# dhillon24/3d-shape-generation

Measured on AMD Instinct MI355X. Metric: denoising-steps/sec (whole node), 2048-pt DDPM, batch 64, higher is better.
Workload: dtype f16; 1 GPU; BASELINE configs[1]: point-cloud DDPM (sample2), 2048 points, batch 64 per GPU, 1000-step cosine schedule, fp16 operands/fp32 accumulate, random-init synthetic weights, denoiser UNetPointNetLarge; batch_per_gpu=64, points=2048, sampler=ddpm/sample2, backbone=pointnet, launch=eager, rccl_ranks=1

## Files before the change

3d-shape-generation_amd/_lib.py:

```python
from __future__ import annotations

import ctypes as C
import os
import subprocess
from typing import Optional

_HERE = os.path.dirname(os.path.abspath(__file__))
LIB_PATH = os.path.join(_HERE, "libpcd_hip.so")
ABI_VERSION = 2
CSRC = os.path.join(_HERE, "csrc")

vp = C.c_void_p
i32, i64, u64, f32, sz = C.c_int, C.c_int64, C.c_uint64, C.c_float, C.c_size_t

PCD_UNET_NLIN = 26


class GemmDesc(C.Structure):
    _fields_ = [("a1", vp), ("lda1", i64), ("k1", i32),
                ("a2", vp), ("lda2", i64), ("k2", i32),
                ("w", vp), ("ldw", i64),
                ("bias", vp), ("shape_bias", vp), ("rows_per_shape", i32),
                ("relu", i32), ("m", i32), ("c", i32)]

# ... 65 lines not shown


class VaeConvT(C.Structure):
    _fields_ = [("w", vp * 8), ("taps", vp * 8), ("b", vp), ("cin", i32), ("cout", i32)]


class VaeDesc(C.Structure):
    _fields_ = [("latent_dim", i32), ("enc0_w", vp), ("enc0_b", vp),
                ("enc_res", VaeRes * 4), ("enc_down", VaeConv * 3), ("enc_last", VaeConv),
                ("fc_w", vp), ("fc_b", vp), ("din_w", vp), ("din_b", vp),
                ("dec_up", VaeConvT * 3), ("dec_res", VaeRes * 4), ("dec_conv9", VaeConv),
                ("last_w", vp), ("last_b", f32),
                ("taps3", vp), ("taps4s2", vp), ("taps4p0", vp), ("taps1", vp), ("zero_page", vp)]


class RenderStyle(C.Structure):
    _fields_ = [("colors", vp), ("light", f32 * 3), ("ambient", f32), ("background", f32 * 3)]


PCD_PAIR_WS = ("an", "bn", "mins", "alpha", "beta", "rowc", "cmax", "err", "bits", "total")


def pair_metrics_workspace_layout(pairs: int, na_max: int, nb_max: int) -> dict:
    off = (sz * len(PCD_PAIR_WS))()
    check(load().pcd_pair_metrics_workspace_layout(pairs, na_max, nb_max, off), "pair_metrics_workspace_layout")
    return dict(zip(PCD_PAIR_WS, (int(v) for v in off)))


PCD_SURF_ROW = ("ACC", "COMP", "CHAMFER_L1", "ACC2", "COMP2", "CHAMFER_L2", "HAUSDORFF", "NC_A", "NC_B", "NC")
PCD_SURF_ROW_BASE = len(PCD_SURF_ROW)
PCD_SURF_MAX_THRESHOLDS = 8
PCD_KNN_MAX_K = 32
PCD_NORMALS_UNORIENTED, PCD_NORMALS_OUTWARD, PCD_NORMALS_TOWARD_VIEW = 0, 1, 2
PCD_OUTLIER_STATISTICAL, PCD_OUTLIER_RADIUS = 0, 1


_SIGS = {
    "pcd_last_error": (C.c_char_p, []),
    "pcd_abi_version": (i32, []),
    "pcd_device_check": (i32, []),
    "pcd_gemm_f16": (i32, [C.POINTER(GemmDesc), vp, i64, vp]),
    "pcd_gemm_f16_hilo": (i32, [C.POINTER(GemmDesc), vp, i64, vp]),
    "pcd_gemm_f16_out32": (i32, [C.POINTER(GemmDesc), vp, i64, vp]),
    "pcd_gemm_f16_splitk": (i32, [C.POINTER(GemmDesc), i32, vp, vp]),
    "pcd_sum_slabs_f32": (i32, [vp, i32, i64, i32, vp, i64, vp]),
    "pcd_gemm_f16_residual": (i32, [C.POINTER(GemmDesc), vp, i64, vp, i64, vp]),
    "pcd_gemm_f16_colmax": (i32, [C.POINTER(GemmDesc), vp, i32, vp]),
    "pcd_gemm_pack_wfrag": (i32, [vp, i64, i32, i32, vp, vp]),
    "pcd_gemm_f16_colmax_wfrag": (i32, [C.POINTER(GemmDesc), vp, vp, i32, vp]),
    "pcd_gemm_wfrag_enabled": (i32, []),
    "pcd_gemm_f16_wfrag": (i32, [C.POINTER(GemmDesc), vp, vp, i64, vp]),
    "pcd_gemm_store_wfrag_enabled": (i32, []),
    "pcd_gemm_wfrag_stamps": (i32, [vp]),
    "pcd_gemm_set_config": (i32, [i32]),
    "pcd_gemm_plan": (i32, [C.POINTER(GemmDesc), i32, i32, i32, i32, C.POINTER(GemmPlan)]),
    "pcd_fill_zero": (i32, [vp, sz, vp]),
    "pcd_f32_to_f16": (i32, [vp, vp, i64, vp]),
    "pcd_f16_to_f32": (i32, [vp, vp, i64, vp]),
    "pcd_time_embed": (i32, [vp, i32, vp, i32, i32, vp, vp, vp, vp, vp, vp, vp, i32, vp, vp]),
    "pcd_linear_f32": (i32, [vp, i32, i32, vp, vp, i32, vp, vp]),
    "pcd_enc1_xyz": (i32, [vp, i64, i32, vp, i32, vp, i32, vp, vp]),
    "pcd_add_noise": (i32, [vp, vp, vp, vp, i32, i64, i64, vp, vp]),
    "pcd_remove_noise": (i32, [vp, vp, vp, vp, i32, i64, i64, vp, vp]),
    "pcd_ddim_update": (i32, [vp, vp, vp, vp, vp, vp, i32, i64, i64, vp, vp, vp]),
    "pcd_ddpm_update": (i32, [vp, vp, vp, vp, vp, vp, vp, i32, i64, i64, vp, vp, vp]),
    "pcd_ddpm_update_philox": (i32, [vp, vp, vp, vp, vp, vp, i32, i64, i64, vp, vp, u64, u64, u64, vp, vp]),
    "pcd_randn": (i32, [vp, i64, u64, u64, vp]),
    "pcd_step_select": (i32, [vp, i32, vp, i32, vp, vp, i32, vp, vp]),
    "pcd_randn_step": (i32, [vp, i64, u64, u64, u64, vp, vp]),
    "pcd_step_select_cols": (i32, [vp, i32, vp, i32, vp, vp, i32, i32, vp, vp]),
    "pcd_step_select_labels": (i32, [vp, i32, vp, i32, vp, vp, i32, vp, i32, i32, vp, i32, i32, vp, vp]),
    "pcd_cfg_combine": (i32, [vp, vp, vp, i32, i64, i64, vp]),
    "pcd_complete_start": (i32, [vp, vp, vp, vp, vp, i32, i64, i64, i32, vp]),
    "pcd_complete_update": (i32, [vp, vp, vp, vp, vp, vp, vp, i32, i32, i64, i64, i32, vp, vp, vp]),
    "pcd_complete_update_philox": (i32, [vp, vp, vp, vp, vp, i32, i32, i64, i64, i32, i32, vp, vp, u64, u64, u64, u64, vp, vp]),
    "pcd_dpm_update": (i32, [vp, vp, vp, i32, i32, i64, i64, vp, vp, vp]),
    "pcd_head3": (i32, [vp, i64, i32, vp, vp, vp, vp]),
    "pcd_pw_chain_enc1": (i32, [vp, i64, i32, vp, vp, i32, vp, vp, vp, vp, vp, vp]),
    "pcd_pw_chain_enc1_hilo": (i32, [vp, i64, i32, vp, vp, i32, vp, vp, vp, vp, vp, vp]),
    "pcd_pw_chain_tail_hilo": (i32, [vp, i64, vp, vp, vp, vp, vp, vp, vp, vp, vp, vp]),
    "pcd_pw_chain_128": (i32, [vp, i64, vp, vp, vp, vp, vp, vp]),
    "pcd_pw_chain_tail": (i32, [vp, i64, vp, vp, vp, vp, vp, vp, vp, vp, vp, vp]),
    "pcd_unet_config": (i32, [i32]),
    "pcd_pw_wide_packed_bytes": (sz, [i32]),
    "pcd_pw_wide_pack": (i32, [i32, vp, vp, vp, vp]),
    "pcd_pw_wide_chain": (i32, [i32, vp, vp, i64, vp, vp, vp]),
    "pcd_pw_wide_ends_packed_bytes": (sz, [i32, i32]),
    "pcd_pw_wide_ends_pack": (i32, [i32, i32, vp, vp, vp, vp]),
    "pcd_pw_wide_ends": (i32, [i32, i32, vp, vp, vp, i64, vp, vp, vp, vp]),
    "pcd_conv1x1_supported": (i32, [i32, i32]),
    "pcd_conv1x1_f16": (i32, [vp, i64, i32, vp, i64, vp, i32, i32, vp, vp]),
    "pcd_unet_create": (i32, [C.POINTER(UnetDesc), C.POINTER(vp)]),
    "pcd_unet_destroy": (None, [vp]),
    "pcd_unet_workspace_bytes": (sz, [i32, i32]),
    "pcd_unet_forward": (i32, [vp, vp, i32, i32, vp, i32, vp, vp, sz, vp]),
    "pcd_unet_profile": (i32, [vp, i32]),
    "pcd_unet_profile_read": (i32, [vp, C.POINTER(C.c_double), C.POINTER(i32)]),
    "pcd_unet_tap": (i32, [vp, C.c_char_p, i32, i32, vp, vp, sz, vp]),
    "pcd_unet_capture": (i32, [vp, vp, vp, vp, vp]),
    "pcd_gemm_f32": (i32, [vp, i64, i32, vp, i64, i32, vp, i64, vp, vp, i32, i32, i32, i32, vp, i64, vp]),
    "pcd_gemm_f32_colmax": (i32, [vp, i64, i32, vp, i64, vp, i32, i32, vp, i32, vp]),
    "pcd_unet_f32_create": (i32, [C.POINTER(UnetDesc), C.POINTER(vp)]),
    "pcd_unet_f32_destroy": (None, [vp]),
    "pcd_unet_f32_workspace_bytes": (sz, [i32, i32]),
    "pcd_unet_f32_forward": (i32, [vp, vp, i32, i32, vp, i32, vp, vp, sz, vp]),
    "pcd_unet_f32_tap": (i32, [vp, C.c_char_p, i32, i32, vp, vp, sz, vp]),
    "pcd_unet_f32_round_activations": (i32, [vp, C.c_uint]),
    "pcd_groupnorm_relu_f16": (i32, [vp, i32, i32, i32, vp, vp, vp, vp]),
    "pcd_skinny_slabs": (i32, [i32, i32]),
    "pcd_skinny_gemm_f16": (i32, [vp, i32, vp, i32, vp, i64, i32, i32, vp, vp]),
    "pcd_skinny_gemm_f32in": (i32, [vp, i32, vp, i64, i32, i32, vp, vp]),
    "pcd_skinny_finish":(i32, [vp, i32, i32, i32, vp, vp, i32, i32, vp, vp, vp, vp, vp]),
    "pcd_skinny_config": (i32, [i32]),
    "pcd_skinny_fused_supported": (i32, [i32, i32, i32, i32]),
    "pcd_skinny_fused": (i32, [vp, i32, vp, i32, vp, i64, i32, i32, vp, vp, i32, i32, vp, vp, vp, vp, vp]),
    "pcd_skinny_fused_f32in": (i32, [vp, i32, vp, i64, i32, i32, vp, vp, i32, i32, vp, vp, vp, vp, vp]),
    "pcd_latent_create": (i32, [C.POINTER(LatentDesc), C.POINTER(vp)]),
    "pcd_latent_destroy": (None, [vp]),
    "pcd_latent_workspace_bytes": (sz, [i32]),
    "pcd_latent_forward": (i32, [vp, vp, i32, vp, i32, vp, vp, sz, vp]),
    "pcd_latent_f32_create": (i32, [C.POINTER(LatentDesc), C.POINTER(vp)]),
    "pcd_latent_f32_destroy": (None, [vp]),
    "pcd_latent_f32_workspace_bytes": (sz, [i32]),
    "pcd_latent_f32_forward": (i32, [vp, vp, i32, vp, i32, vp, vp, sz, vp]),
    "pcd_latent_persist_supported": (i32, [i32]),
    "pcd_latent_persist_create": (i32, [C.POINTER(LatentDesc), C.POINTER(vp)]),
    "pcd_latent_persist_destroy": (None, [vp]),
    "pcd_latent_persist_workspace_bytes": (sz, [vp]),
    "pcd_latent_persist_config": (i32, [vp, i32, i32]),
    "pcd_latent_persist_trace": (i32, [vp, vp, i32]),
    "pcd_latent_persist_forward": (i32, [vp, vp, i32, vp, vp, vp, sz, vp]),
    "pcd_latent_persist_ddim": (i32, [vp, vp, vp, i32, vp, i32, vp, i32, i32, vp, i32, vp, sz, vp]),
    "pcd_latent_persist_status": (i32, [vp, C.POINTER(C.c_uint), vp]),
    "pcd_latent_persist_inject_fault": (i32, [vp, i32, i32]),
    "pcd_latent_persist_plan_check": (i32, []),
    "pcd_latent_persist_plan_dump": (i32, [vp]),
    "pcd_conv3d_f16": (i32, [C.POINTER(Conv3dDesc), vp]),
    "pcd_conv3d_k3s1_supported": (i32, [C.POINTER(Conv3dDesc)]),
    "pcd_conv3d_k3s1_f16": (i32, [C.POINTER(Conv3dDesc), vp]),
    "pcd_conv3d_workspace_bytes": (sz, [C.POINTER(Conv3dDesc), i32]),
    "pcd_conv3d_f16_multi": (i32, [C.POINTER(Conv3dDesc), i32, vp, sz, vp]),
    "pcd_conv3d_wfrag_bytes": (sz, [i32, i32]),
    "pcd_conv3d_pack_wfrag": (i32, [vp, i32, i32, i32, i32, vp, vp]),
    "pcd_conv3d_k3s1_wreg_supported": (i32, [C.POINTER(Conv3dDesc)]),
    "pcd_conv3d_k3s1_wreg_f16": (i32, [C.POINTER(Conv3dDesc), vp, vp]),
    "pcd_conv3d_k4s2_halo_supported": (i32, [i32, i32, i32, i32, i32, i32, i32]),
    "pcd_conv3d_k4s2_halo_f16": (i32, [vp, i32, i32, i32, i32, i32, vp, i32, vp, i32, i32, vp, vp]),
    "pcd_convt3d_k4s2_halo_supported": (i32, [i32, i32, i32, i32, i32, i32]),
    "pcd_convt3d_k4s2_halo_f16": (i32, [vp, i32, i32, i32, i32, i32, C.POINTER(vp), vp, i32, vp, vp]),
    "pcd_conv3d_first": (i32, [vp, i32, i32, i32, i32, i32, vp, vp, i32, vp, vp]),
    "pcd_convt3d_last_sigmoid": (i32, [vp, i32, i32, i32, i32, i32, vp, f32, vp, vp]),
    "pcd_conv3d_config": (i32, [i32]),
    "pcd_conv3d_last_sigmoid": (i32, [vp, i32, i32, i32, i32, i32, vp, f32, vp, vp]),
    "pcd_conv3d_last_packed_bytes": (sz, []),
    "pcd_conv3d_last_pack": (i32, [vp, vp, vp]),
    "pcd_conv3d_last_sigmoid_packed": (i32, [vp, i32, i32, i32, i32, i32, vp, vp, f32, vp, vp]),
    "pcd_reparameterize": (i32, [vp, vp, vp, vp, i64, vp]),
    "pcd_vae_config": (i32, [i32]),
    "pcd_vae_create": (i32, [C.POINTER(VaeDesc), C.POINTER(vp)]),
    "pcd_vae_destroy": (None, [vp]),
    "pcd_vae_workspace_bytes": (sz, [i32]),
    "pcd_vae_encode": (i32, [vp, vp, i32, vp, vp, sz, vp]),
    "pcd_vae_decode": (i32, [vp, vp, i32, vp, vp, sz, vp]),
    "pcd_layernorm_f16": (i32, [vp, i64, i32, vp, vp, vp, vp]),
    "pcd_set_attention_workspace_bytes": (sz, [i32, i32, i32]),
    "pcd_set_attention_f16": (i32, [vp, i32, i32, i32, i32, vp, vp, sz, vp]),
# ... 178 lines not shown
```

3d-shape-generation_amd/csrc/unet.hip:

```cpp
#include <string.h>
#include <new>
#include "common.h"

struct pcd_unet {
    pcd_unet_desc_t d;
    static constexpr int kMaxEv = 4096;
    int prof_on = 0;
    int prof_n = 0;
    hipEvent_t ev0[kMaxEv];
    hipEvent_t ev1[kMaxEv];
    int ev_created = 0;
    void* wide[2] = {nullptr, nullptr};
    void* ends[2] = {nullptr, nullptr};
    void* gf3_frag = nullptr;
    void* lin_frag[PCD_UNET_NLIN] = {};
    void* dec_tap[4] = {nullptr, nullptr, nullptr, nullptr};
};

namespace pcd {

int pw_chain_enc1_impl(const float* x, int64_t m, int rows_per_shape, const float* w_xyz, const float* tbias, int tbias_shape_stride,
                       const void* w_conv2, const float* b_conv2, const void* w_conv3, const float* b_conv3, void* x1, bool hilo,
                       float* zero, int64_t zero_n, void* stream);


struct UnetWs {
    size_t x1, x2, x3, x4, s0, s1, pooled, pooled16, gbias, total;
};

static UnetWs carve(int64_t batch, int64_t n) {
    const size_t m = (size_t)batch * (size_t)n;
    UnetWs w{};
    size_t o = 0;
    w.x1 = o; o += align_up(m * 128 * 2);
    w.x2 = o; o += align_up(m * 256 * 2);
    w.x3 = o; o += align_up(m * 512 * 2);
    w.x4 = o; o += align_up(m * 1024 * 2);
    w.s0 = o; o += align_up(m * 2048 * 2);
    const size_t slabs = batch <= 256 ? (size_t)pcd_skinny_slabs(4096, 1024) * (size_t)batch * 1024 * 4 : 0;
    w.s1 = o; o += align_up(m * 1024 * 2 > slabs ? m * 1024 * 2 : slabs);
    w.pooled = o; o += align_up((size_t)batch * 4096 * 4);
    w.pooled16 = o; if (batch > 256) o += align_up((size_t)batch * 4096 * 2);
    w.gbias = o; o += align_up((size_t)batch * 1024 * 4);
    w.total = o;
    return w;
}

}

using namespace pcd;

static const int kLinK[PCD_UNET_NLIN] = {64, 64, 128, 128, 128, 256, 256, 256, 512, 512, 512, 1024, 2048,
                                         1024, 1024, 1024, 1024, 512, 512, 512, 256, 256, 256, 128, 128, 64};
static const int kLinC[PCD_UNET_NLIN] = {64, 128, 128, 128, 256, 256, 256, 512, 512, 512, 1024, 2048, 4096,
                                         1024, 1024, 512, 512, 512, 256, 256, 256, 128, 128, 128, 64, 64};

static int g_unet_chains = 3;

extern "C" int pcd_unet_config(int use_chains) {
    g_unet_chains = use_chains & 3;
    return PCD_OK;
}

extern "C" int pcd_unet_create(const pcd_unet_desc_t* desc, pcd_unet_t** out) {
    PCD_CHECK_ARG(desc != nullptr && out != nullptr);
    PCD_CHECK_ARG(desc->freqs && desc->tw0 && desc->tb0 && desc->tw2 && desc->tb2);
    PCD_CHECK_ARG(desc->e1w_xyz && desc->e1w_t && desc->e1b && desc->wg && desc->head_w && desc->head_b);
    PCD_CHECK_ARG(desc->wg_k == 4096 && desc->wg_c == 1024);
    if (desc->hilo_mask & ~PCD_UNET_HILO_ALLOWED) {
        set_error("pcd_unet_create: hilo_mask 0x%x names layers outside 0x%x", desc->hilo_mask, PCD_UNET_HILO_ALLOWED);
        return PCD_ERR_ARG;
    }
    for (int i = 0; i < PCD_UNET_NLIN; ++i) {
        if (desc->lin[i].w == nullptr || desc->lin[i].b == nullptr || desc->lin[i].k != kLinK[i] ||
            desc->lin[i].c != kLinC[i]) {
            set_error("pcd_unet_create: layer %d expects %d->%d, got %d->%d (or null pointers)", i, kLinK[i],
                      kLinC[i], desc->lin[i].k, desc->lin[i].c);
            return PCD_ERR_ARG;
        }
    }
    pcd_unet* h = new (std::nothrow) pcd_unet;
    PCD_CHECK_ARG(h != nullptr);
    h->d = *desc;
    const int first[2] = {5, 19};
    for (int c = 0; c < 2; ++c) {
        const void* w[3] = {desc->lin[first[c]].w, desc->lin[first[c] + 1].w, desc->lin[first[c] + 2].w};
        const float* b[3] = {desc->lin[first[c]].b, desc->lin[first[c] + 1].b, desc->lin[first[c] + 2].b};
        hipError_t e = hipMalloc(&h->wide[c], pcd_pw_wide_packed_bytes(c));
        int rc = e == hipSuccess ? pcd_pw_wide_pack(c, w, b, h->wide[c], nullptr) : PCD_ERR_HIP;
        if (rc == PCD_OK && hipStreamSynchronize(nullptr) != hipSuccess) rc = PCD_ERR_HIP;
        if (rc != PCD_OK) {
            if (e != hipSuccess) set_error("pcd_unet_create: %s", hipGetErrorString(e));
            pcd_unet_destroy(h);
            return rc;
        }
    }
    h->gf3_frag = pcd_packed_copy(desc->lin[12].w, (size_t)4096 * 2048 * 2,
                                  [&](void* buf) { return pcd_gemm_pack_wfrag(desc->lin[12].w, 2048, 2048, 4096, buf, nullptr); });
    for (int i = 8; i <= 18; ++i) {
        if (i == 12 || ((desc->hilo_mask >> i) & 1u) || kLinK[i] < 384 || kLinC[i] % 256 != 0) continue;
        h->lin_frag[i] = pcd_packed_copy(desc->lin[i].w, (size_t)kLinK[i] * kLinC[i] * 2,
                                         [&](void* buf) { return pcd_gemm_pack_wfrag(desc->lin[i].w, kLinK[i], kLinK[i], kLinC[i], buf, nullptr); });
    }
    for (int c = 0; c < 2; ++c) {
        const int first = c == 0 ? 2 : 19, nl = c == 0 ? 6 : 4;
        const int hilo = (int)((desc->hilo_mask >> (c == 0 ? 4 : 22)) & 1u);
        const void* w[6]; const float* b[6];
        for (int i = 0; i < nl; ++i) { w[i] = desc->lin[first + i].w; b[i] = desc->lin[first + i].b; }
        h->ends[c] = pcd_packed_copy(w[0], pcd_pw_wide_ends_packed_bytes(c, hilo), [&](void* buf) { return pcd_pw_wide_ends_pack(c, hilo, w, b, buf, nullptr); });
    }
    *out = h;
    return PCD_OK;
}

extern "C" void pcd_unet_destroy(pcd_unet_t* h) {
    if (h == nullptr) return;
    if (h->gf3_frag) (void)hipFree(h->gf3_frag);
    for (int i = 0; i < PCD_UNET_NLIN; ++i) if (h->lin_frag[i]) (void)hipFree(h->lin_frag[i]);
    for (int k = 0; k < 2; ++k) if (h->wide[k]) (void)hipFree(h->wide[k]);
    for (int k = 0; k < 2; ++k) if (h->ends[k]) (void)hipFree(h->ends[k]);
    for (int i = 0; i < h->ev_created; ++i) { (void)hipEventDestroy(h->ev0[i]); (void)hipEventDestroy(h->ev1[i]); }
    delete h;
}

extern "C" int pcd_unet_profile(pcd_unet_t* h, int enable) {
    PCD_CHECK_ARG(h != nullptr);
    h->prof_on = enable ? 1 : 0;
    h->prof_n = 0;
    return PCD_OK;
}

extern "C" int pcd_unet_profile_read(pcd_unet_t* h, double* total_ms, int* launches) {
    PCD_CHECK_ARG(h && total_ms && launches);
    double tot = 0.0;
    for (int i = 0; i < h->prof_n; ++i) {
        PCD_CHECK_HIP(hipEventSynchronize(h->ev1[i]));
        float ms = 0.f;
        PCD_CHECK_HIP(hipEventElapsedTime(&ms, h->ev0[i], h->ev1[i]));
        tot += ms;
    }
    *total_ms = tot;
    *launches = h->prof_n;
    return PCD_OK;
// ... 2 lines not shown
extern "C" int pcd_unet_capture(pcd_unet_t* h, void* d4, void* d3, void* d2, void* d1) {
    PCD_CHECK_ARG(h != nullptr);
    h->dec_tap[0] = d4; h->dec_tap[1] = d3; h->dec_tap[2] = d2; h->dec_tap[3] = d1;
    return PCD_OK;
}

extern "C" size_t pcd_unet_workspace_bytes(int batch, int n_points) {
    if (batch <= 0 || n_points <= 0) return 0;
    return carve(batch, n_points).total;
}

static int run_lin(const pcd_unet_desc_t& d, int idx, int64_t m, const void* a1, const void* a2, int k2,
                   const float* shape_bias, int rps, void* out, hipStream_t s, const void* wfrag = nullptr) {
    pcd_gemm_desc_t g{};
    const pcd_linear_desc_t& L = d.lin[idx];
    g.a1 = a1; g.k1 = L.k - k2; g.lda1 = g.k1;
    g.a2 = a2; g.k2 = k2; g.lda2 = k2;
    const bool hilo = (d.hilo_mask >> idx) & 1u;
    g.w = L.w; g.ldw = hilo ? 2 * L.k : L.k;
    g.bias = shape_bias ? nullptr : L.b;
    g.shape_bias = shape_bias; g.rows_per_shape = rps;
    g.relu = 1; g.m = (int)m; g.c = L.c;
    if (hilo) return pcd_gemm_f16_hilo(&g, out, L.c, s);
    return wfrag != nullptr ? pcd_gemm_f16_wfrag(&g, wfrag, out, L.c, s) : pcd_gemm_f16(&g, out, L.c, s);
}

extern "C" int pcd_unet_forward(pcd_unet_t* h, const float* x, int batch, int n_points, const float* tbias,
                                int tbias_shape_stride, float* eps, void* workspace, size_t workspace_bytes,
                                void* stream) {
    PCD_CHECK_ARG(h && x && tbias && eps && workspace);
    PCD_CHECK_ARG(batch > 0 && n_points > 0);
    const int64_t m = (int64_t)batch * n_points;
    PCD_CHECK_ARG(m <= 0x7fffffff);
    const UnetWs w = carve(batch, n_points);
    if (workspace_bytes < w.total) {
        set_error("pcd_unet_forward: workspace %zu < required %zu", workspace_bytes, w.total);
        return PCD_ERR_WORKSPACE;
    }
    char* ws = (char*)workspace;
    void *x1 = ws + w.x1, *x2 = ws + w.x2, *x3 = ws + w.x3, *x4 = ws + w.x4, *s0 = ws + w.s0, *s1 = ws + w.s1;
    float* pooled = (float*)(ws + w.pooled);
    float* gbias = (float*)(ws + w.gbias);
    hipStream_t s = (hipStream_t)stream;
    const pcd_unet_desc_t& d = h->d;
    int rc;
    const bool chains = (g_unet_chains & 1) != 0;
    bool pooled_cleared = false;
    const bool wide = (g_unet_chains & 2) != 0 && m % 256 == 0;
    const bool e23 = wide && h->ends[0] != nullptr;
    const bool d21 = wide && h->ends[1] != nullptr && h->dec_tap[2] == nullptr;
    if (chains) {
        const unsigned e1 = d.hilo_mask & 3u;
        if (e1 == 3u || e1 == 0u) {
            PCD_RUN(pw_chain_enc1_impl(x, m, n_points, d.e1w_xyz, tbias, tbias_shape_stride, d.lin[0].w, d.lin[0].b, d.lin[1].w, d.lin[1].b, x1,
                                   e1 == 3u, pooled, (int64_t)batch * 4096, s));
            pooled_cleared = true;
        } else {
            PCD_RUN(pcd_enc1_xyz(x, m, n_points, d.e1w_xyz, 64, tbias, tbias_shape_stride, s0, s));
            PCD_RUN(run_lin(d, 0, m, s0, nullptr, 0, nullptr, 0, s1, s));
            PCD_RUN(run_lin(d, 1, m, s1, nullptr, 0, nullptr, 0, x1, s));
        }
        if (!e23) PCD_RUN(pcd_pw_chain_128(x1, m, d.lin[2].w, d.lin[2].b, d.lin[3].w, d.lin[3].b, s1, s));
    } else {
        PCD_RUN(pcd_enc1_xyz(x, m, n_points, d.e1w_xyz, 64, tbias, tbias_shape_stride, s0, s));
        PCD_RUN(run_lin(d, 0, m, s0, nullptr, 0, nullptr, 0, s1, s));
        PCD_RUN(run_lin(d, 1, m, s1, nullptr, 0, nullptr, 0, x1, s));
        if (!e23) {
            PCD_RUN(run_lin(d, 2, m, x1, nullptr, 0, nullptr, 0, s0, s));
            PCD_RUN(run_lin(d, 3, m, s0, nullptr, 0, nullptr, 0, s1, s));
        }
    }
    if (e23) {
        PCD_RUN(pcd_pw_wide_ends(0, (int)((d.hilo_mask >> 4) & 1u), x1, nullptr, nullptr, m, h->ends[0], x3, x2, s));
    } else {
        PCD_RUN(run_lin(d, 4, m, s1, nullptr, 0, nullptr, 0, x2, s));
        if (wide) {
            PCD_RUN(pcd_pw_wide_chain(0, x2, nullptr, m, h->wide[0], x3, s));
        } else {
            PCD_RUN(run_lin(d, 5, m, x2, nullptr, 0, nullptr, 0, s0, s));
            PCD_RUN(run_lin(d, 6, m, s0, nullptr, 0, nullptr, 0, s1, s));
            PCD_RUN(run_lin(d, 7, m, s1, nullptr, 0, nullptr, 0, x3, s));
        }
    }
    PCD_RUN(run_lin(d, 8, m, x3, nullptr, 0, nullptr, 0, s0, s, h->lin_frag[8]));
    PCD_RUN(run_lin(d, 9, m, s0, nullptr, 0, nullptr, 0, s1, s, h->lin_frag[9]));
    PCD_RUN(run_lin(d, 10, m, s1, nullptr, 0, nullptr, 0, x4, s, h->lin_frag[10]));
    PCD_RUN(run_lin(d, 11, m, x4, nullptr, 0, nullptr, 0, s0, s, h->lin_frag[11]));
    {
        if (!pooled_cleared) PCD_RUN(pcd_fill_zero(pooled, (size_t)batch * 4096 * sizeof(float), s));
        pcd_gemm_desc_t g{};
        g.a1 = s0; g.k1 = 2048; g.lda1 = 2048; g.w = d.lin[12].w; g.ldw = 2048; g.bias = d.lin[12].b;
        g.relu = 1; g.m = (int)m; g.c = 4096;
        const bool prof = h->prof_on && h->prof_n < pcd_unet::kMaxEv;
        if (prof) {
            if (h->prof_n >= h->ev_created) {
                PCD_CHECK_HIP(hipEventCreate(&h->ev0[h->ev_created]));
                PCD_CHECK_HIP(hipEventCreate(&h->ev1[h->ev_created]));
                ++h->ev_created;
            }
            PCD_CHECK_HIP(hipEventRecord(h->ev0[h->prof_n], s));
        }
        if (gemm_colmax_takes_wfrag(&g, n_points, h->gf3_frag))
            PCD_RUN(pcd_gemm_f16_colmax_wfrag(&g, h->gf3_frag, pooled, n_points, s));
        else
            PCD_RUN(pcd_gemm_f16_colmax(&g, pooled, n_points, s));
        if (prof) { PCD_CHECK_HIP(hipEventRecord(h->ev1[h->prof_n], s)); ++h->prof_n; }
    }
    {
        if (batch <= 256) {
            PCD_RUN(pcd_skinny_gemm_f32in(pooled, 4096, d.wg, 4096, batch, 1024, (float*)s1, s));
            PCD_RUN(pcd_skinny_finish((const float*)s1, pcd_skinny_slabs(4096, 1024), batch, 1024, d.lin[13].b, nullptr, 2, 8,
                                  nullptr, nullptr, nullptr, gbias, s));
        } else {
            void* pooled16 = ws + w.pooled16;
            PCD_RUN(pcd_f32_to_f16(pooled, pooled16, (int64_t)batch * 4096, s));
            pcd_gemm_desc_t g{};
            g.a1 = pooled16; g.k1 = 4096; g.lda1 = 4096; g.w = d.wg; g.ldw = 4096; g.bias = d.lin[13].b;
            g.relu = 0; g.m = batch; g.c = 1024;
            PCD_RUN(pcd_gemm_f16_out32(&g, gbias, 1024, s));
        }
    }
    PCD_RUN(run_lin(d, 13, m, x4, nullptr, 0, gbias, n_points, s1, s, h->lin_frag[13]));
    PCD_RUN(run_lin(d, 14, m, s1, nullptr, 0, nullptr, 0, s0, s, h->lin_frag[14]));
    PCD_RUN(run_lin(d, 15, m, s0, nullptr, 0, nullptr, 0, s1, s, h->lin_frag[15]));
#define TAP(i, buf, ch) do { if (h->dec_tap[i]) PCD_CHECK_HIP(hipMemcpyAsync(h->dec_tap[i], buf, (size_t)m * (ch) * 2, \
                                                                             hipMemcpyDeviceToDevice, s)); } while (0)
    TAP(0, s1, 512);
    PCD_RUN(run_lin(d, 16, m, s1, x3, 512, nullptr, 0, s0, s, h->lin_frag[16]));
    PCD_RUN(run_lin(d, 17, m, s0, nullptr, 0, nullptr, 0, s1, s, h->lin_frag[17]));
    PCD_RUN(run_lin(d, 18, m, s1, nullptr, 0, nullptr, 0, s0, s, h->lin_frag[18]));
    TAP(1, s0, 256);
    void *ta = s0, *tb = s1;
    if (d21) {
        PCD_RUN(pcd_pw_wide_ends(1, (int)((d.hilo_mask >> 22) & 1u), s0, x2, x1, m, h->ends[1], s1, nullptr, s));
        ta = s1; tb = s0;
    } else {
        if (wide) {
            PCD_RUN(pcd_pw_wide_chain(1, s0, x2, m, h->wide[1], s1, s));
        } else {
            PCD_RUN(run_lin(d, 19, m, s0, x2, 256, nullptr, 0, s1, s));
            PCD_RUN(run_lin(d, 20, m, s1, nullptr, 0, nullptr, 0, s0, s));
            PCD_RUN(run_lin(d, 21, m, s0, nullptr, 0, nullptr, 0, s1, s));
        }
        TAP(2, s1, 128);
        PCD_RUN(run_lin(d, 22, m, s1, x1, 128, nullptr, 0, s0, s));
    }
    const unsigned tl = (d.hilo_mask >> 23) & 7u;
    if (chains && h->dec_tap[3] == nullptr && (tl == 0u || tl == 7u)) {
        if (tl == 7u)
            PCD_RUN(pcd_pw_chain_tail_hilo(ta, m, d.lin[23].w, d.lin[23].b, d.lin[24].w, d.lin[24].b, d.lin[25].w, d.lin[25].b, d.head_w,
                                       d.head_b, eps, s));
        else
            PCD_RUN(pcd_pw_chain_tail(ta, m, d.lin[23].w, d.lin[23].b, d.lin[24].w, d.lin[24].b, d.lin[25].w, d.lin[25].b, d.head_w,
                                  d.head_b, eps, s));
    } else {
        PCD_RUN(run_lin(d, 23, m, ta, nullptr, 0, nullptr, 0, tb, s));
        PCD_RUN(run_lin(d, 24, m, tb, nullptr, 0, nullptr, 0, ta, s));
        TAP(3, ta, 64);
        PCD_RUN(run_lin(d, 25, m, ta, nullptr, 0, nullptr, 0, tb, s));
        PCD_RUN(pcd_head3(tb, m, 64, d.head_w, d.head_b, eps, s));
    }
#undef TAP
    return PCD_OK;
}

extern "C" int pcd_unet_tap(pcd_unet_t* h, const char* name, int batch, int n_points, const void* workspace,
                            void* dst, size_t dst_bytes, void* stream) {
    PCD_CHECK_ARG(h && name && workspace && dst && batch > 0 && n_points > 0);
    const UnetWs w = carve(batch, n_points);
    const size_t m = (size_t)batch * n_points;
    size_t off = 0, bytes = 0;
    if (!strcmp(name, "x1")) { off = w.x1; bytes = m * 128 * 2; }
    else if (!strcmp(name, "x2")) { off = w.x2; bytes = m * 256 * 2; }
    else if (!strcmp(name, "x3")) { off = w.x3; bytes = m * 512 * 2; }
    else if (!strcmp(name, "x4")) { off = w.x4; bytes = m * 1024 * 2; }
    else if (!strcmp(name, "pooled")) { off = w.pooled; bytes = (size_t)batch * 4096 * 4; }
    else if (!strcmp(name, "gbias")) { off = w.gbias; bytes = (size_t)batch * 1024 * 4; }
    else { set_error("pcd_unet_tap: unknown tap '%s'", name); return PCD_ERR_ARG; }
    PCD_CHECK_ARG(dst_bytes >= bytes);
    PCD_CHECK_HIP(hipMemcpyAsync(dst, (const char*)workspace + off, bytes, hipMemcpyDeviceToDevice, (hipStream_t)stream));
    return PCD_OK;
}
```

include/pcd_hip.h:

```cpp
#ifndef PCD_HIP_H
#define PCD_HIP_H

#include <stddef.h>
#include <stdint.h>

#ifdef __cplusplus
extern "C" {
#endif

#define PCD_OK 0
#define PCD_ERR_ARG (-1)
#define PCD_ERR_HIP (-2)
#define PCD_ERR_WORKSPACE (-3)

#define PCD_ABI_VERSION 2

const char* pcd_last_error(void);
int pcd_abi_version(void);
int pcd_device_check(void);

typedef struct {
    const void* a1; int64_t lda1; int k1;
    const void* a2; int64_t lda2; int k2;
    const void* w;  int64_t ldw;
// ... 48 lines not shown
                   float* y, void* stream);

int pcd_enc1_xyz(const float* x, int64_t m, int rows_per_shape, const float* w_xyz, int c1,
                 const float* tbias, int tbias_shape_stride, void* out, void* stream);

int pcd_add_noise(const float* x0, const float* noise, const float* n, const float* s, int stride,
                  int64_t total, int64_t per_shape, float* x_t, void* stream);
int pcd_remove_noise(const float* x_t, const float* eps, const float* n, const float* s, int stride,
                     int64_t total, int64_t per_shape, float* x0, void* stream);
int pcd_ddim_update(const float* x, const float* eps, const float* n, const float* s,
                    const float* n2, const float* s2, int stride,
                    int64_t total, int64_t per_shape, float* x0, float* x_next, void* stream);
int pcd_ddpm_update(const float* x, const float* eps, const float* z, const float* n, const float* s,
                    const float* coef, const float* s2, int stride,
                    int64_t total, int64_t per_shape, float* x0, float* x_next, void* stream);
int pcd_ddpm_update_philox(const float* x, const float* eps, const float* n, const float* s, const float* coef, const float* s2,
                           int stride, int64_t total, int64_t per_shape, float* x0, float* x_next, uint64_t seed,
                           uint64_t base_offset, uint64_t per_step_stride, const int* counter, void* stream);
int pcd_randn(float* out, int64_t n, uint64_t seed, uint64_t offset, void* stream);

int pcd_step_select(int* counter, int n_steps, const float* tb_table, int tb_elems, float* tb_cur,
                    const float* rate_tables, int width, float* rates_cur, void* stream);
int pcd_randn_step(float* out, int64_t n, uint64_t seed, uint64_t base_offset, uint64_t per_step_stride,
                   const int* counter, void* stream);
int pcd_step_select_cols(int* counter, int n_steps, const float* tb_table, int tb_elems, float* tb_cur,
                         const float* rate_tables, int cols, int width, float* rates_cur, void* stream);

int pcd_step_select_labels(int* counter, int n_steps, const float* tb_table, int tb_elems, float* tb_rows,
                           const float* class_bias, int class_rows, const int* labels, int batch, int null_row,
                           const float* rate_tables, int cols, int width, float* rates_cur, void* stream);
int pcd_cfg_combine(float* eps, const float* eps_u, const float* w, int w_stride, int64_t n, int64_t per_shape, void* stream);

int pcd_complete_start(float* x, const float* p, const int* counts, const float* n, const float* s, int stride,
                       int64_t total, int64_t per_shape, int row_elems, void* stream);
int pcd_complete_update(const float* x, const float* eps, const float* z, const float* z2, const float* p,
                        const int* counts, const float* rates, int width, int stride, int64_t total,
                        int64_t per_shape, int row_elems, float* x0, float* x_next, void* stream);
int pcd_complete_update_philox(const float* x, const float* eps, const float* p, const int* counts,
                               const float* rates, int width, int stride, int64_t total, int64_t per_shape,
                               int row_elems, int jumps, float* x0, float* x_next, uint64_t seed,
                               uint64_t base_offset, uint64_t per_step_stride, uint64_t z2_offset,
                               const int* counter, void* stream);

int pcd_dpm_update(const float* x, const float* eps, const float* rates, int width, int stride, int64_t total,
                   int64_t per_shape, float* hist, float* x_next, void* stream);

int pcd_head3(const void* h, int64_t m, int k, const float* w, const float* b, float* eps, void* stream);

#define PCD_UNET_NLIN 26
typedef struct {
    const void* w; const float* b; int k; int c;
} pcd_linear_desc_t;

typedef struct {
    int time_dim, dim;
    const float* freqs;
    const float *tw0, *tb0, *tw2, *tb2;
    const float* e1w_xyz;
    const float* e1w_t;
    const float* e1b;
    pcd_linear_desc_t lin[PCD_UNET_NLIN];
    const void* wg; int wg_k, wg_c;
    const float* head_w; const float* head_b;
    unsigned hilo_mask;
} pcd_unet_desc_t;
#define PCD_UNET_HILO_ALLOWED 0x3C00013u

int pcd_pw_chain_enc1(const float* x, int64_t m, int rows_per_shape, const float* w_xyz, const float* tbias,
                      int tbias_shape_stride, const void* w_conv2, const float* b_conv2, const void* w_conv3,
                      const float* b_conv3, void* x1, void* stream);
int pcd_pw_chain_128(const void* in, int64_t m, const void* w_a, const float* b_a, const void* w_b, const float* b_b,
                     void* out, void* stream);
int pcd_pw_chain_tail(const void* in, int64_t m, const void* w_a, const float* b_a, const void* w_b, const float* b_b,
                      const void* w_c, const float* b_c, const float* head_w, const float* head_b, float* eps, void* stream);
int pcd_pw_chain_enc1_hilo(const float* x, int64_t m, int rows_per_shape, const float* w_xyz, const float* tbias,
                           int tbias_shape_stride, const void* w_conv2, const float* b_conv2, const void* w_conv3,
                           const float* b_conv3, void* x1, void* stream);
int pcd_pw_chain_tail_hilo(const void* in, int64_t m, const void* w_a, const float* b_a, const void* w_b, const float* b_b,
                           const void* w_c, const float* b_c, const float* head_w, const float* head_b, float* eps, void* stream);
int pcd_conv1x1_supported(int k, int c);
int pcd_conv1x1_f16(const void* in, int64_t m, int k, const void* w, int64_t ldw, const float* bias, int relu, int c,
                    void* out, void* stream);
int pcd_unet_config(int use_chains);
size_t pcd_pw_wide_packed_bytes(int chain);
int pcd_pw_wide_pack(int chain, const void* const* w, const float* const* b, void* packed, void* stream);
int pcd_pw_wide_chain(int chain, const void* in1, const void* in2, int64_t m, const void* packed, void* out, void* stream);
int pcd_pw_wide_config(int split);
size_t pcd_pw_wide_ends_packed_bytes(int chain, int hilo);
int pcd_pw_wide_ends_pack(int chain, int hilo, const void* const* w, const float* const* b, void* packed, void* stream);
int pcd_pw_wide_ends(int chain, int hilo, const void* in1, const void* in2, const void* in3, int64_t m, const void* packed, void* out, void* out2,
                     void* stream);
size_t pcd_pw_wide_ln_linear_packed_bytes(int passes);
int pcd_pw_wide_ln_linear_pack(const void* w, const float* b, int passes, const float* ln_g, const float* ln_b, void* packed, void* stream);
int pcd_pw_wide_ln_linear_supported(int dim, int64_t rows);
int pcd_pw_wide_ln_linear(const void* packed, int passes, int relu, const void* x, int64_t rows, void* out, void* stream);

typedef struct pcd_unet pcd_unet_t;
int pcd_unet_create(const pcd_unet_desc_t* desc, pcd_unet_t** out);
void pcd_unet_destroy(pcd_unet_t* h);
size_t pcd_unet_workspace_bytes(int batch, int n_points);
int pcd_unet_forward(pcd_unet_t* h, const float* x, int batch, int n_points,
                     const float* tbias, int tbias_shape_stride,
                     float* eps, void* workspace, size_t workspace_bytes, void* stream);
int pcd_unet_profile(pcd_unet_t* h, int enable);
int pcd_unet_profile_read(pcd_unet_t* h, double* total_ms, int* launches);
int pcd_unet_tap(pcd_unet_t* h, const char* name, int batch, int n_points,
                 const void* workspace, void* dst, size_t dst_bytes, void* stream);
int pcd_unet_capture(pcd_unet_t* h, void* d4, void* d3, void* d2, void* d1);

int pcd_gemm_f32(const float* a1, int64_t lda1, int k1, const float* a2, int64_t lda2, int k2, const float* w, int64_t ldw,
                 const float* bias, const float* shape_bias, int rows_per_shape, int relu, int m, int c, float* out,
                 int64_t ldo, void* stream);
int pcd_gemm_f32_colmax(const float* a, int64_t lda, int k, const float* w, int64_t ldw, const float* bias, int m, int c,
                        float* pooled, int rows_per_shape, void* stream);
typedef struct pcd_unet_f32 pcd_unet_f32_t;
int pcd_unet_f32_create(const pcd_unet_desc_t* desc, pcd_unet_f32_t** out);
void pcd_unet_f32_destroy(pcd_unet_f32_t* h);
size_t pcd_unet_f32_workspace_bytes(int batch, int n_points);
int pcd_unet_f32_forward(pcd_unet_f32_t* h, const float* x, int batch, int n_points, const float* tbias,
                         int tbias_shape_stride, float* eps, void* workspace, size_t workspace_bytes, void* stream);
int pcd_unet_f32_round_activations(pcd_unet_f32_t* h, unsigned mask);
int pcd_unet_f32_tap(pcd_unet_f32_t* h, const char* name, int batch, int n_points, const void* workspace, void* dst,
                     size_t dst_bytes, void* stream);

int pcd_groupnorm_relu_f16(const float* x, int rows, int c, int groups, const float* gamma,
                           const float* beta, void* out, void* stream);
int pcd_skinny_slabs(int k, int c);
int pcd_skinny_gemm_f16(const void* a1, int k1, const void* a2, int k2, const void* w, int64_t ldw,
                        int m, int c, float* slabs, void* stream);
int pcd_skinny_gemm_f32in(const float* a, int k, const void* w, int64_t ldw, int m, int c, float* slabs, void* stream);
int pcd_skinny_finish(const float* slabs, int nslabs, int m, int c, const float* bias, const float* row_bias,
                      int mode, int groups, const float* gamma, const float* beta,
                      void* out16, float* out32, void* stream);
int pcd_skinny_config(int use_lds_dma);
int pcd_skinny_fused_supported(int k, int c, int mode, int groups);
int pcd_skinny_fused(const void* a1, int k1, const void* a2, int k2, const void* w, int64_t ldw, int m, int c,
                     const float* bias, const float* row_bias, int mode, int groups, const float* gamma,
                     const float* beta, void* out16, float* out32, void* stream);
int pcd_skinny_fused_f32in(const float* a, int k, const void* w, int64_t ldw, int m, int c, const float* bias,
                           const float* row_bias, int mode, int groups, const float* gamma, const float* beta,
                           void* out16, float* out32, void* stream);
#define PCD_LATENT_NLIN 12
typedef struct {
    pcd_linear_desc_t lin[PCD_LATENT_NLIN];
    const float* gn_gamma[PCD_LATENT_NLIN];
    const float* gn_beta[PCD_LATENT_NLIN];
} pcd_latent_desc_t;
typedef struct pcd_latent pcd_latent_t;
int pcd_latent_create(const pcd_latent_desc_t* desc, pcd_latent_t** out);
void pcd_latent_destroy(pcd_latent_t* h);
size_t pcd_latent_workspace_bytes(int batch);
int pcd_latent_forward(pcd_latent_t* h, const float* z, int batch, const float* tbias,
                       int tbias_shape_stride, float* eps, void* workspace, size_t workspace_bytes,
                       void* stream);

typedef struct pcd_latent_f32 pcd_latent_f32_t;
int pcd_latent_f32_create(const pcd_latent_desc_t* desc, pcd_latent_f32_t** out);
void pcd_latent_f32_destroy(pcd_latent_f32_t* h);
size_t pcd_latent_f32_workspace_bytes(int batch);
int pcd_latent_f32_forward(pcd_latent_f32_t* h, const float* z, int batch, const float* tbias, int tbias_shape_stride,
                           float* eps, void* workspace, size_t workspace_bytes, void* stream);

typedef struct pcd_latent_persist pcd_latent_persist_t;
int pcd_latent_persist_supported(int batch);
int pcd_latent_persist_create(const pcd_latent_desc_t* desc, pcd_latent_persist_t** out);
void pcd_latent_persist_destroy(pcd_latent_persist_t* h);
// ... 349 lines not shown
```

Measured before the change: 280.9 denoising-steps/sec.

## Fuse encoder and decoder pointwise layer chains into persistent LDS panel kernels

```diff
diff --git a/3d-shape-generation_amd/_lib.py b/3d-shape-generation_amd/_lib.py
--- a/3d-shape-generation_amd/_lib.py
+++ b/3d-shape-generation_amd/_lib.py
@@ -171,6 +171,7 @@
     "pcd_pw_chain_128": (i32, [vp, i64, vp, vp, vp, vp, vp, vp]),
     "pcd_pw_chain_tail": (i32, [vp, i64, vp, vp, vp, vp, vp, vp, vp, vp, vp, vp]),
     "pcd_unet_config": (i32, [i32]),
+    "pcd_panel_chain": (i32, [i32, vp, i64, vp, vp, i32, vp, i64, i32, vp]),
     "pcd_pw_wide_packed_bytes": (sz, [i32]),
     "pcd_pw_wide_pack": (i32, [i32, vp, vp, vp, vp]),
     "pcd_pw_wide_chain": (i32, [i32, vp, vp, i64, vp, vp, vp]),
diff --git a/3d-shape-generation_amd/csrc/panelchain.hip b/3d-shape-generation_amd/csrc/panelchain.hip
--- /dev/null
+++ b/3d-shape-generation_amd/csrc/panelchain.hip
@@ -0,0 +1,281 @@
+#include <type_traits>
+#include "common.h"
+
+namespace pcd {
+
+namespace {
+
+constexpr int PC_ROWS = 128, PC_K = 512, PC_NK = 8, PC_THREADS = 512;
+constexpr int PC_PANEL = PC_ROWS * PC_K * 2;
+constexpr int PC_SLOTS = 8 * 2048;
+constexpr int PC_MAXL = 3;
+
+struct PcPass { int layer, col0, two_by_four, store; };
+struct PcChain { int nlayers, c[PC_MAXL], npass; PcPass pass[4]; int c_out; };
+constexpr PcChain PC_CHAIN[2] = {
+    {3, {512, 512, 1024}, 4, {{0, 0, 0, 0}, {1, 0, 0, 0}, {2, 0, 0, 1}, {2, 512, 0, 1}}, 1024},
+    {2, {512, 256, 0}, 2, {{0, 0, 0, 0}, {1, 0, 1, 1}, {0, 0, 0, 0}, {0, 0, 0, 0}}, 256},
+};
+constexpr int pc_bias_off(int chain, int layer) {
+    int o = 0;
+    for (int l = 0; l < layer; ++l) o += PC_CHAIN[chain].c[l];
+    return o;
+}
+constexpr int pc_lds_bytes(int chain) { return PC_PANEL + PC_SLOTS + pc_bias_off(chain, PC_CHAIN[chain].nlayers) * 4; }
+
+struct PcParams {
+    const half_t* x;
+    const half_t* frag[PC_MAXL];
+    const float* bias[PC_MAXL];
+    half_t* out; int ldo;
+    int tiles;
+};
+
+typedef unsigned u32x4_t __attribute__((ext_vector_type(4)));
+
+__device__ __forceinline__ const half_t* pc_uniform(const half_t* q) {
+    const uint64_t v = (uint64_t)q;
+    return (const half_t*)(((uint64_t)(unsigned)__builtin_amdgcn_readfirstlane((int)(v >> 32)) << 32) | (unsigned)__builtin_amdgcn_readfirstlane((int)v));
+}
+__device__ __forceinline__ void pc_dma16(unsigned voff, const half_t* sbase, unsigned lds_addr) {
+    asm volatile("s_mov_b32 m0, %2\n\ts_nop 0\n\tglobal_load_lds_dwordx4 %0, %1" ::"v"(voff), "s"(sbase), "s"(lds_addr) : "memory", "m0");
+}
+__device__ __forceinline__ void pc_store16(unsigned voff, u32x4_t data, const half_t* sbase) {
+    asm volatile("global_store_dwordx4 %0, %1, %2\n\ts_nop 1" ::"v"(voff), "v"(data), "s"(sbase) : "memory");
+}
+__device__ __forceinline__ void pc_relu_pack(const f32x4 v, unsigned (&pk)[2]) {
+    half2_ lo2, hi2;
+    lo2[0] = (half_t)__builtin_amdgcn_fmed3f(v[0], 0.f, 65504.f);
+    lo2[1] = (half_t)__builtin_amdgcn_fmed3f(v[1], 0.f, 65504.f);
+    hi2[0] = (half_t)__builtin_amdgcn_fmed3f(v[2], 0.f, 65504.f);
+    hi2[1] = (half_t)__builtin_amdgcn_fmed3f(v[3], 0.f, 65504.f);
+    pk[0] = __builtin_bit_cast(unsigned, lo2);
+    pk[1] = __builtin_bit_cast(unsigned, hi2);
+}
+
+template <int CHAIN>
+__global__ __launch_bounds__(PC_THREADS) void panel_chain_kernel(PcParams p) {
+    constexpr PcChain CH = PC_CHAIN[CHAIN];
+    constexpr int NP = CH.npass;
+    constexpr int NI = 4;
+    extern __shared__ __attribute__((aligned(16))) char lds[];
+    char* const panel = lds;
+    float* const bias_lds = reinterpret_cast<float*>(lds + PC_PANEL + PC_SLOTS);
+    const int tid = threadIdx.x;
+    const int lane = tid & 63;
+    const int wave = __builtin_amdgcn_readfirstlane(tid >> 6);
+
+    int tile = __builtin_amdgcn_readfirstlane((int)blockIdx.x);
+    if (tile >= p.tiles) return;
+
+#pragma unroll
+    for (int l = 0; l < CH.nlayers; ++l)
+        for (int i = tid; i < CH.c[l]; i += PC_THREADS) bias_lds[pc_bias_off(CHAIN, l) + i] = p.bias[l][i];
+    __syncthreads();
+
+    const unsigned vlane16 = (unsigned)(lane * 16);
+    auto request_panel = [&](int t) __attribute__((always_inline)) {
+        unsigned l16 = vlane16;
+        asm volatile("" : "+v"(l16));
+        const unsigned r8 = l16 >> 7, c8 = (l16 >> 4) & 7;
+#pragma unroll
+        for (int h = 0; h < 2; ++h) {
+            const unsigned voff = r8 * (PC_K * 2) + ((c8 ^ ((4 * h + (r8 >> 1)) & 7)) << 4);
+            const half_t* g = pc_uniform(p.x + ((int64_t)t * PC_ROWS + wave * 16 + h * 8) * PC_K);
+            const unsigned dst = (unsigned)(size_t)panel + (unsigned)((wave * 2 + h) * 1024);
+#pragma unroll
+            for (int kt = 0; kt < PC_NK; ++kt) pc_dma16(voff, g + kt * 64, dst + kt * 16384);
+        }
+    };
+    auto pass_weights = [&](auto pc) __attribute__((always_inline)) {
+        constexpr int P = decltype(pc)::value;
+        constexpr PcPass D = CH.pass[P];
+        const int tn = D.col0 / 256 + (D.two_by_four ? 0 : (wave >> 2));
+        return pc_uniform(p.frag[D.layer] + ((int64_t)tn * PC_NK * 4 + (wave & 3)) * 4096);
+    };
+    auto wload = [&](const half_t* wks, auto jc) __attribute__((always_inline)) {
+        constexpr int J = decltype(jc)::value;
+        half8 v;
+        asm volatile("global_load_dwordx4 %0, %1, %2 offset:%3" : "=v"(v) : "v"(vlane16), "s"(wks), "n"(J * 1024) : "memory");
+        return v;
+    };
+    auto wload4 = [&](half8 (&dst)[NI], const half_t* wks) __attribute__((always_inline)) {
+        dst[0] = wload(wks, std::integral_constant<int, 0>{});
+        dst[1] = wload(wks, std::integral_constant<int, 1>{});
+        dst[2] = wload(wks, std::integral_constant<int, 2>{});
+        dst[3] = wload(wks, std::integral_constant<int, 3>{});
+    };
+
+    char* const slot = lds + PC_PANEL + wave * 2048;
+
+    f32x4 acc[8][NI];
+    half8 wq[2][NI];
+
+    request_panel(tile);
+    {
+        const half_t* w0 = pass_weights(std::integral_constant<int, 0>{});
+        wload4(wq[0], w0);
+        wload4(wq[1], w0 + 2048);
+    }
+    wait_vmcnt<0>();
+    __builtin_amdgcn_s_barrier();
+
+    for (;;) {
+        const int next = tile + (int)gridDim.x;
+        const bool has_next = next < p.tiles;
+
+        auto run_pass = [&](auto pc) __attribute__((always_inline)) {
+            constexpr int P = decltype(pc)::value;
+            constexpr PcPass D = CH.pass[P];
+            constexpr int PN = (P + 1) % NP, PP = (P + NP - 1) % NP;
+            constexpr int MI = D.two_by_four ? 4 : 8;
+            constexpr int NST_PREV = CH.pass[PP].store ? (CH.pass[PP].two_by_four ? 8 : 16) : 0;
+            const int row0 = D.two_by_four ? (wave >> 2) * 64 : 0;
+            const int wcol = D.two_by_four ? (wave & 3) : wave;
+            const half_t* wcur = pass_weights(pc);
+            const half_t* wnp = pass_weights(std::integral_constant<int, PN>{});
+#pragma unroll
+            for (int i = 0; i < MI; ++i)
+#pragma unroll
+                for (int j = 0; j < NI; ++j) acc[i][j] = (f32x4){0.f, 0.f, 0.f, 0.f};
+            int offa[2];
+            {
+                unsigned l16 = vlane16;
+                asm volatile("" : "+v"(l16));
+                const int pr = (l16 >> 4) & 15, q = l16 >> 8;
+#pragma unroll
+                for (int ks = 0; ks < 2; ++ks) offa[ks] = pr * 128 + (((ks * 4 + q) ^ ((pr >> 1) & 7)) << 4);
+            }
+            auto k_tile = [&](int kt, auto waitc) __attribute__((always_inline)) {
+                constexpr int WAITC = decltype(waitc)::value;
+                int ktv = kt;
+                asm volatile("" : "+s"(ktv));
+                const half_t* wnext = pc_uniform(ktv + 1 < PC_NK ? wcur + (int64_t)(ktv + 1) * 16384 : wnp);
+                const char* base = panel + ktv * 16384 + row0 * 128;
+#pragma unroll
+                for (int ks = 0; ks < 2; ++ks) {
+                    half8 af[MI];
+#pragma unroll
+                    for (int i = 0; i < MI; ++i) af[i] = *(const half8*)(base + offa[ks] + i * 2048);
+                    wait_vmcnt<WAITC>();
+                    __builtin_amdgcn_s_setprio(1);
+#pragma unroll
+                    for (int i = 0; i < MI; ++i)
+#pragma unroll
+                        for (int j = 0; j < NI; ++j) acc[i][j] = __builtin_amdgcn_mfma_f32_16x16x32_f16(wq[ks][j], af[i], acc[i][j], 0, 0, 0);
+                    __builtin_amdgcn_s_setprio(0);
+                    __builtin_amdgcn_sched_barrier(0);
+                    wload4(wq[ks], wnext + ks * 2048);
+                    __builtin_amdgcn_sched_barrier(0);
+                }
+            };
+            if constexpr (NST_PREV > 0) k_tile(0, std::integral_constant<int, 4 + NST_PREV>{});
+#pragma unroll 1
+            for (int kt = NST_PREV > 0 ? 1 : 0; kt < PC_NK; ++kt) k_tile(kt, std::integral_constant<int, 4>{});
+            unsigned l16 = vlane16;
+            asm volatile("" : "+v"(l16));
+            const int pr = (l16 >> 4) & 15, q = l16 >> 8;
+            const int seg = 2 * (q & 1) + (q >> 1);
+            f32x4 bv[NI];
+#pragma unroll
+            for (int j = 0; j < NI; ++j) bv[j] = *(const f32x4*)&bias_lds[pc_bias_off(CHAIN, D.layer) + D.col0 + wcol * 64 + j * 16 + q * 4];
+            if constexpr (!D.store) {
+                const int hand_off = wave * 16384 + pr * 128 + ((seg ^ ((pr >> 1) & 7)) << 4);
+                wait_lgkm0();
+                __builtin_amdgcn_s_barrier();
+#pragma unroll
+                for (int i = 0; i < MI; ++i)
+#pragma unroll
+                    for (int j = 0; j < NI; j += 2) {
+                        unsigned pk[2][2];
+                        pc_relu_pack(acc[i][j] + bv[j], pk[0]);
+                        pc_relu_pack(acc[i][j + 1] + bv[j + 1], pk[1]);
+                        const auto s0 = __builtin_amdgcn_permlane16_swap(pk[0][0], pk[1][0], false, false);
+                        const auto s1 = __builtin_amdgcn_permlane16_swap(pk[0][1], pk[1][1], false, false);
+                        const u32x4_t o = {s0[0], s1[0], s0[1], s1[1]};
+                        *(u32x4_t*)(panel + ((hand_off ^ ((j >> 1) * 64)) + i * 2048)) = o;
+                    }
+                wait_lgkm0();
+                __builtin_amdgcn_s_barrier();
+            } else {
+                constexpr bool LAST = P + 1 == NP;
+                if constexpr (LAST) {
+                    wait_lgkm0();
+                    __builtin_amdgcn_s_barrier();
+                    if (has_next) request_panel(next);
+                }
+                const int slot_wr = pr * 128 + ((seg ^ (pr & 7)) << 4);
+                const int slot_rd = (l16 >> 7) * 128 + ((((l16 >> 4) & 7) ^ (l16 >> 7)) << 4);
+                const unsigned vline = (unsigned)(((l16 >> 7) * p.ldo + ((l16 >> 4) & 7) * 8) * 2);
+                const half_t* orow = p.out + ((int64_t)tile * PC_ROWS + row0) * p.ldo + D.col0 + wcol * 64;
+#pragma unroll
+                for (int i = 0; i < MI; ++i) {
+#pragma unroll
+                    for (int j = 0; j < NI; j += 2) {
+                        unsigned pk[2][2];
+                        pc_relu_pack(acc[i][j] + bv[j], pk[0]);
+                        pc_relu_pack(acc[i][j + 1] + bv[j + 1], pk[1]);
+                        const auto s0 = __builtin_amdgcn_permlane16_swap(pk[0][0], pk[1][0], false, false);
+                        const auto s1 = __builtin_amdgcn_permlane16_swap(pk[0][1], pk[1][1], false, false);
+                        const u32x4_t o = {s0[0], s1[0], s0[1], s1[1]};
+                        *(u32x4_t*)(slot + (slot_wr ^ ((j >> 1) * 64))) = o;
+                    }
+#pragma unroll
+                    for (int h = 0; h < 2; ++h) {
+                        const u32x4_t dv = *(const u32x4_t*)(slot + h * 1024 + slot_rd);
+                        pc_store16(vline, dv, pc_uniform(orow + (int64_t)(i * 16 + h * 8) * p.ldo));
+                    }
+                }
+                if constexpr (LAST) {
+                    if (has_next) {
+                        wait_vmcnt<D.two_by_four ? 8 : 16>();
+                        __builtin_amdgcn_s_barrier();
+                    }
+                }
+            }
+        };
+        run_pass(std::integral_constant<int, 0>{});
+        run_pass(std::integral_constant<int, 1>{});
+        if constexpr (NP > 2) run_pass(std::integral_constant<int, 2>{});
+        if constexpr (NP > 3) run_pass(std::integral_constant<int, 3>{});
+        if (!has_next) break;
+        tile = next;
+    }
+    wait_vmcnt<0>();
+#pragma unroll
+    for (int ks = 0; ks < 2; ++ks)
+#pragma unroll
+        for (int j = 0; j < NI; ++j) asm volatile("" ::"v"(wq[ks][j]));
+}
+
+}
+
+}
+
+using namespace pcd;
+
+extern "C" int pcd_panel_chain(int chain, const void* x, int64_t m, const void* const* frag, const float* const* bias, int hilo, void* out, int64_t ld,
+                               int cap, void* stream) {
+    PCD_CHECK_ARG(chain == 0 || chain == 1);
+    PCD_CHECK_ARG(x != nullptr && frag != nullptr && bias != nullptr && out != nullptr && x != out);
+    PCD_CHECK_ARG(m > 0 && m % PC_ROWS == 0 && m <= 0x7fffffff);
+    PCD_CHECK_ARG(cap >= 1 && cap <= 256);
+    PCD_CHECK_ARG(hilo == 0);
+    const PcChain& ch = PC_CHAIN[chain];
+    PCD_CHECK_ARG(ld >= ch.c_out && ld % 8 == 0 && (7 * ld + 64) * 2 < 0x7fffffffLL);
+    PcParams p{};
+    for (int l = 0; l < ch.nlayers; ++l) {
+        PCD_CHECK_ARG(frag[l] != nullptr && bias[l] != nullptr);
+        p.frag[l] = (const half_t*)frag[l]; p.bias[l] = bias[l];
+    }
+    p.x = (const half_t*)x; p.out = (half_t*)out; p.ldo = (int)ld; p.tiles = (int)(m / PC_ROWS);
+    static PcdLdsOnce once[2];
+    const void* kernel = chain == 0 ? (const void*)panel_chain_kernel<0> : (const void*)panel_chain_kernel<1>;
+    const int lds = pc_lds_bytes(chain);
+    PCD_CHECK_HIP(pcd_allow_lds(once[chain], kernel, lds));
+    const dim3 grid((unsigned)(p.tiles < cap ? p.tiles : cap));
+    if (chain == 0) hipLaunchKernelGGL(panel_chain_kernel<0>, grid, dim3(PC_THREADS), lds, (hipStream_t)stream, p);
+    else hipLaunchKernelGGL(panel_chain_kernel<1>, grid, dim3(PC_THREADS), lds, (hipStream_t)stream, p);
+    PCD_CHECK_LAUNCH();
+    return PCD_OK;
+}
diff --git a/3d-shape-generation_amd/csrc/unet.hip b/3d-shape-generation_amd/csrc/unet.hip
--- a/3d-shape-generation_amd/csrc/unet.hip
+++ b/3d-shape-generation_amd/csrc/unet.hip
@@ -58,7 +58,7 @@
 static int g_unet_chains = 3;
 
 extern "C" int pcd_unet_config(int use_chains) {
-    g_unet_chains = use_chains & 3;
+    g_unet_chains = use_chains & 7;
     return PCD_OK;
 }
 
@@ -227,9 +227,23 @@
             PCD_RUN(run_lin(d, 7, m, s1, nullptr, 0, nullptr, 0, x3, s));
         }
     }
-    PCD_RUN(run_lin(d, 8, m, x3, nullptr, 0, nullptr, 0, s0, s, h->lin_frag[8]));
-    PCD_RUN(run_lin(d, 9, m, s0, nullptr, 0, nullptr, 0, s1, s, h->lin_frag[9]));
-    PCD_RUN(run_lin(d, 10, m, s1, nullptr, 0, nullptr, 0, x4, s, h->lin_frag[10]));
+    const bool panel = (g_unet_chains & 6) == 2 && m % 128 == 0;
+    auto panel_chain = [&](int chain, int first, int nl, const void* in, void* out, int ld) {
+        const void* frag[3]; const float* bias[3];
+        for (int i = 0; i < nl; ++i) { frag[i] = h->lin_frag[first + i]; bias[i] = d.lin[first + i].b; }
+        return pcd_panel_chain(chain, in, m, frag, bias, 0, out, ld, 256, s);
+    };
+    auto has_frags = [&](int first, int nl) {
+        for (int i = first; i < first + nl; ++i) if (h->lin_frag[i] == nullptr || ((d.hilo_mask >> i) & 1u)) return false;
+        return true;
+    };
+    if (panel && has_frags(8, 3)) {
+        PCD_RUN(panel_chain(0, 8, 3, x3, x4, 1024));
+    } else {
+        PCD_RUN(run_lin(d, 8, m, x3, nullptr, 0, nullptr, 0, s0, s, h->lin_frag[8]));
+        PCD_RUN(run_lin(d, 9, m, s0, nullptr, 0, nullptr, 0, s1, s, h->lin_frag[9]));
+        PCD_RUN(run_lin(d, 10, m, s1, nullptr, 0, nullptr, 0, x4, s, h->lin_frag[10]));
+    }
     PCD_RUN(run_lin(d, 11, m, x4, nullptr, 0, nullptr, 0, s0, s, h->lin_frag[11]));
     {
         if (!pooled_cleared) PCD_RUN(pcd_fill_zero(pooled, (size_t)batch * 4096 * sizeof(float), s));
@@ -272,8 +286,13 @@
                                                                              hipMemcpyDeviceToDevice, s)); } while (0)
     TAP(0, s1, 512);
     PCD_RUN(run_lin(d, 16, m, s1, x3, 512, nullptr, 0, s0, s, h->lin_frag[16]));
-    PCD_RUN(run_lin(d, 17, m, s0, nullptr, 0, nullptr, 0, s1, s, h->lin_frag[17]));
-    PCD_RUN(run_lin(d, 18, m, s1, nullptr, 0, nullptr, 0, s0, s, h->lin_frag[18]));
+    if (panel && has_frags(17, 2)) {
+        PCD_RUN(panel_chain(1, 17, 2, s0, s1, 256));
+        void* t = s0; s0 = s1; s1 = t;
+    } else {
+        PCD_RUN(run_lin(d, 17, m, s0, nullptr, 0, nullptr, 0, s1, s, h->lin_frag[17]));
+        PCD_RUN(run_lin(d, 18, m, s1, nullptr, 0, nullptr, 0, s0, s, h->lin_frag[18]));
+    }
     TAP(1, s0, 256);
     void *ta = s0, *tb = s1;
     if (d21) {
diff --git a/include/pcd_hip.h b/include/pcd_hip.h
--- a/include/pcd_hip.h
+++ b/include/pcd_hip.h
@@ -154,6 +154,8 @@
 int pcd_conv1x1_f16(const void* in, int64_t m, int k, const void* w, int64_t ldw, const float* bias, int relu, int c,
                     void* out, void* stream);
 int pcd_unet_config(int use_chains);
+int pcd_panel_chain(int chain, const void* x, int64_t m, const void* const* frag, const float* const* bias, int hilo, void* out, int64_t ld, int cap,
+                    void* stream);
 size_t pcd_pw_wide_packed_bytes(int chain);
 int pcd_pw_wide_pack(int chain, const void* const* w, const float* const* b, void* packed, void* stream);
 int pcd_pw_wide_chain(int chain, const void* in1, const void* in2, int64_t m, const void* packed, void* out, void* stream);
```

Result: faster. 287.6 denoising-steps/sec (median of 6 runs) (+2.4%).
